# KrainskiL/CGE.jl

Measured on AMD Instinct MI355X. Metric: edge_alpha_evals_per_sec, higher is better.
Workload: dtype f64

## Files before the change

### cge.jl_amd/api.py

```python
from __future__ import annotations

import atexit
import ctypes as C
import os
import sys
import weakref

import numpy as np

from .args import _SplitRule

_HERE = os.path.dirname(os.path.abspath(__file__))
_LIB_PATH = os.path.join(_HERE, "csrc", "build", "libcge_hip.so")
_lib = None

CGE_OK = 0
_CODES = {-1: "AssertionError", -2: "ErrorException: Trying to split homogenous cluster",
          -3: "ErrorException: Unexpected empty cluster generated", -4: "HIP error / no GPU",
          -5: "collective hook failed", -6: "out of memory", -7: "bad argument"}


class CGEError(RuntimeError):
    def __init__(self, code, msg=""):
        super().__init__(f"{_CODES.get(code, 'error')} (code {code}){': ' + msg if msg else ''}")
# ... 991 lines not shown
    def set_collectives(self, fn, rank, world):
        cb = ALLREDUCE_FN(fn)
        coll = Collectives(cb, None, rank, world)
        self._keep = [cb, coll]
        self._check(self.L.cge_set_collectives(self.h, C.byref(coll)))

    def set_collectives_ext(self, allgather=None, reduce_scatter=None):
        ag = GATHER_FN(allgather) if allgather else GATHER_FN()
        rs = GATHER_FN(reduce_scatter) if reduce_scatter else GATHER_FN()
        ext = CollectivesExt(ag, rs)
        self._keep = list(getattr(self, "_keep", [])) + [ag, rs, ext]
        self._check(self.L.cge_set_collectives_ext(self.h, C.byref(ext)))

    def clear_collectives(self):
        self._check(self.L.cge_comm_finalize(self.h))
        self._check(self.L.cge_set_collectives(self.h, None))
        self._keep = []

    def init_rccl(self, unique_id: bytes, rank: int, world: int):
        assert len(unique_id) == 128
        buf = C.create_string_buffer(bytes(unique_id), 128)
        self._check(self.L.cge_comm_init_rccl(self.h, buf, C.c_int(rank), C.c_int(world)))

    def finalize_rccl(self):
        self._check(self.L.cge_comm_finalize(self.h))

    def rccl_selftest(self, arr, op=0):
        a = np.ascontiguousarray(arr).copy()
        assert a.dtype.itemsize == 8
        self._check(self.L.cge_rccl_selftest(self.h, _p(a), C.c_int64(a.size), C.c_int(op)))
        return a

    def louvain(self):
        out = np.zeros(self.n, dtype=np.int64)
        nc, q, rounds = C.c_int64(), C.c_double(), C.c_int64()
        self._check(self.L.cge_louvain(self.h, _p(out), C.byref(nc), C.byref(q), C.byref(rounds)))
        return out, nc.value, q.value, rounds.value

    def louvain_levels(self, max_levels=0):
        count, cap = C.c_int64(), (int(max_levels) if 0 < int(max_levels) < 8 else 8)
        while True:
            comm = np.zeros((cap, self.n), dtype=np.int64)
            nc, q, rounds = np.zeros(cap, dtype=np.int64), np.zeros(cap), np.zeros(cap, dtype=np.int64)
            rc = self.L.cge_louvain_levels(self.h, C.c_int64(int(max_levels)), C.c_int64(cap), _p(comm), C.byref(count), _p(nc),
                                           _p(q), _p(rounds))
            if rc == -7 and count.value > cap:
                cap = count.value
                continue
            self._check(rc)
            break
        return [(comm[l], int(nc[l]), float(q[l]), int(rounds[l])) for l in range(count.value)]

    _TEST_OPTIONS = ("louvain_wave_len", "fit_persistent_test_delay", "fit_persistent_test_timeout", "test_bvec_plain", "test_rss2_one_kernel",
                     "exact_resident_limit")

    def set_option(self, key, value):
        if key in self._TEST_OPTIONS:
            self._check(self.L.cge_set_test_option(self.h, key.encode(), C.c_int64(int(value))))
            return
        self._check(self.L.cge_set_option(self.h, key.encode(), C.c_int64(int(value))))

    def get_stat(self, key):
        v = C.c_int64()
        self._check(self.L.cge_get_stat(self.h, key.encode(), C.byref(v)))
        return v.value

    def last_diameter(self):
        import struct

        hi = struct.unpack("d", struct.pack("q", self.get_stat("diameter_bits")))[0]
        return hi, {1: "brute", 2: "pruned"}.get(self.get_stat("diameter_path"), "none"), \
            self.get_stat("diameter_candidate_pairs"), self.get_stat("diameter_candidate_tiles")

    def profile_enable(self, on=True):
        self._check(self.L.cge_profile_enable(self.h, C.c_int(int(on))))

    def profile_select(self, names=()):
        self._check(self.L.cge_profile_select(self.h, ",".join(names).encode()))

    def profile_reset(self):
        self._check(self.L.cge_profile_reset(self.h))

    def profile(self):
        buf = C.create_string_buffer(4096)
        self._check(self.L.cge_profile_names(self.h, buf, C.c_int64(4096)))
        res = {}
        for name in filter(None, buf.value.decode().split(",")):
            n, ms = C.c_int64(), C.c_double()
            self._check(self.L.cge_profile_get(self.h, name.encode(), C.byref(n), C.byref(ms)))
            res[name] = {"launches": n.value, "total_ms": ms.value}
        return res

    def phase_ms(self):
        res = {}
        buf = C.create_string_buffer(4096)
        self._check(self.L.cge_phase_names(self.h, buf, C.c_int64(4096)))
        for ph in filter(None, buf.value.decode().split(",")):
            ms = C.c_double()
            self._check(self.L.cge_phase_ms(self.h, ph.encode(), C.byref(ms)))
            res[ph] = ms.value
        return res


_default_ctx = None


def default_context():
# ... 96 lines not shown
```

### cge.jl_amd/csrc/capi.cpp

```cpp
#include "common.hpp"
#include "../../include/cge_hip_testing.h"

void flush_timers(cge_ctx *c) {
    for (auto &kv : c->timers) {
        for (auto &pr : kv.second.pending) {
            float ms = 0.f;
            (void)hipEventSynchronize(pr.second);
            if (hipEventElapsedTime(&ms, pr.first, pr.second) == hipSuccess) kv.second.total_ms += ms;
            c->event_pool.push_back(pr.first);
            c->event_pool.push_back(pr.second);
        }
        kv.second.pending.clear();
    }
}
template <class Map>
static int key_names(const Map &m, char *buf, int64_t buf_len) {
    std::string s;
    for (auto &kv : m) s += (s.empty() ? "" : ",") + kv.first;
    snprintf(buf, (size_t)buf_len, "%s", s.c_str());
    return CGE_OK;
}

extern "C" {

// ... 230 lines not shown
int cge_louvain(cge_ctx *c, int64_t *comm_out, int64_t *n_comm, double *modularity, int64_t *rounds) {
    if (!c || !comm_out) return CGE_E_ARG;
    CGE_TRY_ON_DEVICE(c)
    if (!c->src.p || c->m <= 0 || c->n <= 0) CGE_THROW(CGE_E_ARG, "louvain: no resident graph (cge_set_graph)");
    if (c->edges_sharded) CGE_THROW(CGE_E_ARG, "louvain: the resident edge list is sharded over the ranks (option shard_ingest)");
    k_louvain_level1(c, comm_out, n_comm, modularity, rounds);
    CGE_CATCH(c)
}
int cge_louvain_levels(cge_ctx *c, int64_t max_levels, int64_t levels_cap, int64_t *comm_out, int64_t *n_levels, int64_t *n_comm,
                       double *modularity, int64_t *rounds) {
    if (!c || !n_levels || levels_cap < 0) return CGE_E_ARG;
    if (levels_cap > 0 && (!comm_out || !n_comm || !modularity || !rounds)) return CGE_E_ARG;
    CGE_TRY_ON_DEVICE(c)
    if (!c->src.p || c->m <= 0 || c->n <= 0) CGE_THROW(CGE_E_ARG, "louvain: no resident graph (cge_set_graph)");
    if (c->edges_sharded) CGE_THROW(CGE_E_ARG, "louvain: the resident edge list is sharded over the ranks (option shard_ingest)");
    *n_levels = k_louvain_levels(c, max_levels, levels_cap, comm_out, n_comm, modularity, rounds);
    if (levels_cap > 0 && *n_levels > levels_cap)
        CGE_THROW(CGE_E_ARG, "louvain: the hierarchy has %lld levels, the caller's arrays hold %lld", (long long)*n_levels,
                  (long long)levels_cap);
    CGE_CATCH(c)
}

int cge_set_option(cge_ctx *c, const char *key, int64_t value) {
    if (!c || !key) return CGE_E_ARG;
    const auto is = [&](const char *k) { return !strcmp(key, k); };
    const auto ranged = [&](auto &field, int64_t lo, int64_t hi) {
        if (value < lo || value > hi) return (int)CGE_E_ARG;
        field = (std::remove_reference_t<decltype(field)>)value;
        return (int)CGE_OK;
    };
    const auto flag = [&](auto &field) { field = value != 0; return (int)CGE_OK; };
    if (is("diameter")) return ranged(c->opt_diameter, 0, 2);
    if (is("diameter_f32")) return ranged(c->opt_diameter_f32, 0, 2);
    if (is("fit_persistent")) return ranged(c->opt_fit_persistent, 0, 2);
    if (is("pow_exp2")) return flag(c->opt_pow_exp2);
    if (is("shard_runsplit")) return ranged(c->opt_shard_forced, 0, 2);
    if (is("shard_samples")) return ranged(c->opt_shard_samples, 0, 2);
    if (is("exact_relabel")) return flag(c->opt_exact_relabel);
    if (is("bvec_blocks")) return flag(c->opt_bvec_blocks);
    if (is("wedges_reduce_scatter")) return flag(c->opt_wedges_rs);
    if (is("fit_fused")) return flag(c->opt_fit_fused);
    if (is("shard_ingest")) return flag(c->opt_shard_ingest);
    if (is("shard_rows")) return flag(c->opt_shard_rows);
    if (is("landmark_edges")) return flag(c->opt_landmark_edges);
    if (is("exact_packed")) return ranged(c->opt_exact_packed, 0, 1);
    if (is("fit_max_iterations")) return ranged(c->opt_fit_max_iters, 1, INT64_MAX);
    return CGE_E_ARG;
}
int cge_set_test_option(void *ctx, const char *key, int64_t value) {
    cge_ctx *c = (cge_ctx *)ctx;
    if (!c || !key) return CGE_E_ARG;
    if (!strcmp(key, "test_bvec_plain")) { c->opt_test_bvec_plain = value != 0; return CGE_OK; }
    if (!strcmp(key, "test_rss2_one_kernel")) { c->opt_test_rss2_one_kernel = value != 0; return CGE_OK; }
    if (!strcmp(key, "fit_persistent_test_delay") && value >= 0 && value <= 100000) { c->opt_fit_test_delay = (int)value; return CGE_OK; }
    if (!strcmp(key, "fit_persistent_test_timeout")) { c->opt_fit_test_timeout = value != 0; return CGE_OK; }
    if (!strcmp(key, "louvain_wave_len") && value >= -2 && value <= INT32_MAX) { c->opt_test_louvain_wave_len = value; return CGE_OK; }
    if (!strcmp(key, "exact_resident_limit") && value >= 0) { c->opt_test_resident_limit = (double)value; return CGE_OK; }
    return CGE_E_ARG;
}
int cge_get_stat(cge_ctx *c, const char *key, int64_t *value) {
    if (!c || !key || !value) return CGE_E_ARG;
    if (!strcmp(key, "landmarks")) *value = c->lm_ready ? c->N : 0;
    else if (!strcmp(key, "diameter_path")) *value = c->stat_diameter_path;
    else if (!strcmp(key, "diameter_candidate_pairs")) *value = c->stat_cand_pairs;
    else if (!strcmp(key, "diameter_candidate_tiles")) *value = c->stat_cand_tiles;
    else if (!strcmp(key, "diameter_refs")) *value = c->stat_nref;
    else if (!strcmp(key, "diameter_bound_pass")) *value = c->stat_bound_pass;
    else if (!strcmp(key, "diameter_arg_i")) *value = c->stat_hi_i + 1;
    else if (!strcmp(key, "diameter_arg_j")) *value = c->stat_hi_j + 1;
    else if (!strcmp(key, "fit_persistent_alphas")) *value = c->stat_fit_persistent;
    else if (!strcmp(key, "fit_iterations")) *value = c->stat_fit_iters;
    else if (!strcmp(key, "exact_packed")) *value = c->stat_exact_packed;
    else if (!strcmp(key, "exact_matrix_bytes")) *value = c->stat_exact_matrix_bytes;
    else if (!strcmp(key, "fit_fused_alphas")) *value = c->stat_fit_fused;
    else if (!strcmp(key, "fit_persistent_fallbacks")) *value = c->stat_fit_fallbacks;
    else if (!strcmp(key, "fit_batched_launches")) *value = c->stat_fit_batched_launches;
    else if (!strcmp(key, "fit_batched_alphas")) *value = c->stat_fit_batched_alphas;
    else if (!strcmp(key, "landmark_batches")) *value = c->stat_lm_batches;
    else if (!strcmp(key, "landmark_batch_rows")) *value = c->stat_lm_rows;
    else if (!strcmp(key, "landmark_splits")) *value = c->stat_lm_splits;
    else if (!strcmp(key, "cut_tie_tasks")) {
        int v = 0;
        if (c->cut_ties.p && (hipStreamSynchronize(c->stream) != hipSuccess ||
                              hipMemcpy(&v, c->cut_ties.p, sizeof(int), hipMemcpyDeviceToHost) != hipSuccess))
            return CGE_E_HIP;
        *value = v;
    }
    else if (!strcmp(key, "edge_layout_build_us")) *value = c->stat_layout_build_us;
    else if (!strcmp(key, "edge_chunks")) *value = c->be_nchunks;
    else if (!strcmp(key, "edges_resident")) *value = c->m;
    else if (!strcmp(key, "edges_total")) *value = c->m_total;
    else if (!strcmp(key, "embedding_words_resident")) *value = (i64)c->Xr.n;
    else if (!strcmp(key, "rows_resident")) *value = c->Xr.p ? lm_rows(c) : 0;
    else if (!strcmp(key, "rows_total")) *value = c->n;
    else if (!strcmp(key, "collective_calls")) *value = c->stat_coll_calls;
    else if (!strcmp(key, "collective_bytes")) *value = c->stat_coll_bytes;
    else if (!strcmp(key, "diameter_bits")) memcpy(value, &c->stat_last_hi, sizeof(double));
    else return CGE_E_ARG;
    return CGE_OK;
}

int cge_profile_enable(cge_ctx *c, int on) {
    if (!c) return CGE_E_ARG;
    c->profiling = on != 0;
    return CGE_OK;
}
// ... 254 lines not shown
```

### cge.jl_amd/csrc/common.hpp

```cpp
#pragma once
#include <hip/hip_runtime.h>

#include <algorithm>
#include <atomic>
#include <chrono>
#include <condition_variable>
#include <functional>
#include <mutex>
#include <thread>
#include <cstdint>
#include <cstdio>
#include <cstdlib>
#include <cstring>
#include <map>
#include <memory>
#include <string>
#include <vector>

#include "../../include/cge_hip.h"

typedef int64_t i64;
typedef int32_t i32;

struct MaxRec {
// ... 298 lines not shown
    DevBuf<double> lemb;
    DevBuf<double> lweight, dii;
    DevBuf<i32> lcomm;
    DevBuf<double> wedges;
    DevBuf<double> vectC;
    i64 n_ledges = 0;
    bool wedges_ready = false;

    DevBuf<double> s_emb, s_dist, s_vw, s_vectC, s_degin, s_degout;
    DevBuf<i32> s_comm;
    DevBuf<double> auc_part, js_part;
    DevBuf<unsigned> js_counter;
    unsigned js_launches = 0;
    DevBuf<double> sw_D, sw_GD, sw_T1, sw_T2, sw_S1, sw_S2, sw_rowbins, sw_vectB, sw_scal, sw_lohi, sw_fitstate, sw_mm;
    DevBuf<int> sw_flags;
    DevBuf<unsigned long long> sw_fring;
    DevBuf<double> sw_PK;
    int opt_exact_packed = 0;
    double opt_test_resident_limit = 0;
    i64 stat_exact_packed = 0;
    i64 stat_exact_matrix_bytes = 0;
    bool sweep_used_fp_P = false;
    DevBuf<double> fp_T, fp_Tsave, fp_P, fp_fpart, fp_Td, fp_flow;
    DevBuf<double> ls_eigscr;
    bool bvec_contig = false;
    bool bvec_blocks = false;
    int opt_bvec_blocks = 0;
    DevBuf<i32> sw_bt_fc, sw_bt_ns, sw_bt_base;
    i64 flow_armed_words = 0;
    DevBuf<double> sw_bt_part;
    DevBuf<i32> sw_bt_desc;
    DevBuf<double> sw_fused_pw;
    DevBuf<char> sw_fused_epi;
    int opt_fit_fused = 1;
    i64 stat_fit_fused = 0;
    DevBuf<double> batch_scal, batch_vectB, batch_jspart, batch_flow;
    PinBuf<double> batch_pin;
    i64 stat_fit_batched_launches = 0, stat_fit_batched_alphas = 0;
    DevBuf<i32> sw_rl_order, sw_rl_comm;
    DevBuf<double> sw_rl_emb, sw_rl_vec, sw_rl_T;
    DevBuf<int> fp_flags;
    PinBuf<double> pin_scal;
    hipEvent_t sweep_ev[2] = {nullptr, nullptr};
    int opt_pow_exp2 = 1;
    i64 pow_logs_N = 0;
    bool pow_logs_upper = false;
    i64 pow_logs_blocked_N = 0;
    DevBuf<double> sw_Lh;
    DevBuf<float> sw_Ll;
    bool opt_exact_relabel = true;
    int opt_shard_samples = 1;
    int opt_shard_forced = 1;
    int opt_test_rss2_one_kernel = 0;
    i64 opt_test_louvain_wave_len = -2;
    int opt_test_bvec_plain = 0;
    int opt_fit_persistent = 0;
    i64 opt_fit_max_iters = 2000000;
    int opt_fit_test_timeout = 0;
    int opt_fit_test_delay = 0;
    i64 stat_lm_batches = 0, stat_lm_rows = 0, stat_lm_splits = 0;
    DevBuf<int> cut_ties;
    i64 stat_fit_persistent = 0;
    i64 stat_fit_iters = 0;
    bool fit_persistent_broken = false;
    i64 stat_fit_fallbacks = 0;
    int fit_fallback_streak = 0;
    i64 fit_skip_sweeps = 0;
    DevBuf<i32> sw_cm_off, sw_cm_mem, sw_cm_pos;
    DevBuf<double> sw_zeros, sw_zsum;
    DevBuf<MaxRec> mp_recs;
    DevBuf<i64> mp_count;
    DevBuf<int2> nt_pairs, nt_tiles;
    DevBuf<i32> nt_idx;
    DevBuf<double> nt_out, nt_rows;
    DevBuf<double> mp_rd2, mp_refmu;
    DevBuf<double> mp_commax;
    DevBuf<int2> mp_plist;
    DevBuf<i32> mp_lref, mp_refoff, mp_refmem;
    DevBuf<double> gmean;
    bool emb_nonfinite = false;
    DevBuf<double> Xs, rns, Ms, mnorm, Pm;
    DevBuf<double> pc_groups;
    DevBuf<float> Xs32, Ms32;
    DevBuf<unsigned short> Xb16, Mb16;
    DevBuf<int> dm_flag;
    DevBuf<double> xe, xe_rns, dm_seed;
    DevBuf<i32> xe_pos, xe_glob, xe_sub, dm_soffE;
    int opt_diameter_f32 = 2;
    DevBuf<i32> pos2node, sub_land, dm_soff, dm_memoff, dm_mem;
    DevBuf<BoundRec> bound_list;
    DevBuf<int2> tile_list;
    std::vector<i32> h_mem_off, h_mem;
    DevBuf<uint64_t> uniq_hash;
    DevBuf<unsigned long long> uniq_table;
    int opt_diameter = 0;
    i64 stat_cand_pairs = 0, stat_cand_tiles = 0;
    int stat_diameter_path = 0;
    double stat_last_hi = 0.0;
    i64 stat_hi_i = -1, stat_hi_j = -1;
    int stat_bound_pass = 0;
    i64 stat_nref = 0;
    DevBuf<i32> ls_rows, ls_row_task, ls_ct, ls_cb, ls_ce, ls_co, ls_tco;
    DevBuf<double> ls_part, ls_mean, ls_sw, ls_cov, ls_vec, ls_z, ls_sums;
    DevBuf<unsigned char> ls_side, ls_state;
    DevBuf<double> ls_params;
    PinBuf<double> pin_sums, pin_params;
// ... 557 lines not shown
```

### cge.jl_amd/csrc/kernels_lm.hip

```cpp
#include "common.hpp"
#include <type_traits>
#include "mfma_tile.hpp"

#define WAVE 64

template <int CTRL>
__device__ __forceinline__ double dpp_move(double v) {
    const long long b = __double_as_longlong(v);
    const int lo = __builtin_amdgcn_update_dpp(0, (int)(unsigned)b, CTRL, 0xf, 0xf, false);
    const int hi = __builtin_amdgcn_update_dpp(0, (int)(unsigned)(b >> 32), CTRL, 0xf, 0xf, false);
    return __longlong_as_double(((long long)hi << 32) | (unsigned)lo);
}
__device__ __forceinline__ double lane_value(double v, int lane) {
    const long long b = __double_as_longlong(v);
    const int lo = __builtin_amdgcn_readlane((int)(unsigned)b, lane);
    const int hi = __builtin_amdgcn_readlane((int)(unsigned)(b >> 32), lane);
    return __longlong_as_double(((long long)hi << 32) | (unsigned)lo);
}
__device__ __forceinline__ double wave_allsum(double v) {
    v += dpp_move<0xB1>(v);
    v += dpp_move<0x4E>(v);
    v += dpp_move<0x141>(v);
    v += dpp_move<0x140>(v);
    return ((lane_value(v, 0) + lane_value(v, 16)) + lane_value(v, 32)) + lane_value(v, 48);
// ... 1764 lines not shown
    asm volatile("v_fmac_f64_dpp %0, %1, -%2 row_newbcast:%3 row_mask:0xf bank_mask:0xf" : "+v"(acc) : "v"(bc), "v"(a), "n"(N));
}
template <int NG>
__device__ __forceinline__ void dpp_fence(double (&v)[NG]) {
    if constexpr (NG == 1) asm volatile("s_nop 1" : "+v"(v[0]));
    else asm volatile("s_nop 1" : "+v"(v[0]), "+v"(v[NG - 1]));
}
template <int JJ, int NR, int NC, int R0 = 0>
struct EigCols {
    static constexpr int NG = (NC + 15) / 16;
    static __device__ __forceinline__ void matvec(double (&s)[NR], const double (&a)[NR][NC], const double (&uc)[NG]) {
#pragma unroll
        for (int r = R0; r < NR; r++) fmac_bcast<JJ % 16>(s[r], uc[JJ / 16], a[r][JJ]);
        EigCols<JJ + 1, NR, NC, R0>::matvec(s, a, uc);
    }
    static __device__ __forceinline__ void rank2(double (&a)[NR][NC], const double (&uc)[NG], const double (&wc)[NG],
                                                 const double (&u)[NR], const double (&w)[NR]) {
#pragma unroll
        for (int r = R0; r < NR; r++) {
            fnmac_bcast<JJ % 16>(a[r][JJ], uc[JJ / 16], w[r]);
            fnmac_bcast<JJ % 16>(a[r][JJ], wc[JJ / 16], u[r]);
        }
        EigCols<JJ + 1, NR, NC, R0>::rank2(a, uc, wc, u, w);
    }
};
template <int NR, int NC, int R0>
struct EigCols<NC, NR, NC, R0> {
    static constexpr int NG = (NC + 15) / 16;
    static __device__ __forceinline__ void matvec(double (&)[NR], const double (&)[NR][NC], const double (&)[NG]) {}
    static __device__ __forceinline__ void rank2(double (&)[NR][NC], const double (&)[NG], const double (&)[NG], const double (&)[NR],
                                                 const double (&)[NR]) {}
};
template <int NR, int NC>
__device__ __forceinline__ void eig_pick_column(const double (&a)[NR][NC], int jj, double (&v)[NR]) {
#define EP_CASE(J)                                                                                                          \
    case J:                                                                                                                 \
        if constexpr (J < NC) {                                                                                             \
            _Pragma("unroll") for (int r = 0; r < NR; r++) v[r] = a[r][J];                                                  \
        }                                                                                                                   \
        break;
#pragma unroll
    for (int r = 0; r < NR; r++) v[r] = 0.0;
    switch (jj) {
        EP_CASE(0) EP_CASE(1) EP_CASE(2) EP_CASE(3) EP_CASE(4) EP_CASE(5) EP_CASE(6) EP_CASE(7)
        EP_CASE(8) EP_CASE(9) EP_CASE(10) EP_CASE(11) EP_CASE(12) EP_CASE(13) EP_CASE(14) EP_CASE(15)
        EP_CASE(16) EP_CASE(17) EP_CASE(18) EP_CASE(19) EP_CASE(20) EP_CASE(21) EP_CASE(22) EP_CASE(23)
        EP_CASE(24) EP_CASE(25) EP_CASE(26) EP_CASE(27) EP_CASE(28) EP_CASE(29) EP_CASE(30) EP_CASE(31)
    default: break;
    }
#undef EP_CASE
}
template <int NR, int NC, bool DPPF>
__global__ __launch_bounds__(256, 2) void group_eig_kernel(const double *__restrict__ cov, int d,
                                                           double *__restrict__ vec, int diag_stage) {
    constexpr int DP = 64 * NR;
    __shared__ __attribute__((aligned(16))) double X[DP], U[DP], W[DP], Pp[4][DP], V[DP];
    __shared__ __attribute__((aligned(16))) double diag[DP], off[DP], beta[DP], V0[DP], tri[4 * DP], red[32];
    const int tid = threadIdx.x, lane = tid & 63, wv = __builtin_amdgcn_readfirstlane(tid >> 6);
    const double *src = cov + (size_t)blockIdx.x * d * d;
    double *out = vec + (size_t)blockIdx.x * d;
    if (d == 1) {
        if (tid == 0) out[0] = 1.0;
        return;
    }
    double a[NR][NC];
#pragma unroll
    for (int r = 0; r < NR; r++) {
        const int row = lane + 64 * r;
#pragma unroll
        for (int jj = 0; jj < NC; jj++) {
            const int col = NC * wv + jj;
            a[r][jj] = (row < d && col < d) ? src[(size_t)col * d + row] : 0.0;
        }
    }
    auto extract = [&](int kn, auto) {
        if (wv == kn / NC) {
            double v[NR];
            eig_pick_column<NR, NC>(a, kn % NC, v);
#pragma unroll
            for (int r = 0; r < NR; r++) X[lane + 64 * r] = v[r];
        }
    };
    using RBlk0 = std::integral_constant<int, 0>;
    using RBlkL = std::integral_constant<int, NR - 1>;
    if (tid < DP) { beta[tid] = 0.0; off[tid] = 0.0; V0[tid] = 0.0; X[tid] = 0.0; }
    __syncthreads();
    extract(0, RBlk0{});
#ifdef CGE_EIG_CLOCK
    unsigned long long ck_acc[8] = {0, 0, 0, 0, 0, 0, 0, 0}, ck_t = __builtin_amdgcn_s_memtime();
#define CK(j) { const unsigned long long ck_n = __builtin_amdgcn_s_memtime(); ck_acc[j] += ck_n - ck_t; ck_t = ck_n; }
#else
#define CK(j)
#endif
    auto hh_step = [&](const int k, auto r0c) {
        constexpr int R0 = decltype(r0c)::value;
        asm volatile("s_waitcnt lgkmcnt(0)" ::: "memory");
        __syncthreads();
        CK(0)
        const int o = k + 1;
        double x[NR], u[NR];
        double part = 0.0;
#pragma unroll
        for (int r = 0; r < NR; r++) {
            const int row = lane + 64 * r;
            x[r] = (row > k) ? X[row] : 0.0;
            part += (row > o) ? x[r] * x[r] : 0.0;
        }
        constexpr int NG = (NC + 15) / 16;
        double uc[NG], wc[NG];
        if (DPPF) {
#pragma unroll
            for (int g = 0; g < NG; g++) {
                const int col = NC * wv + 16 * g + (lane & 15);
                uc[g] = (col > k && col < DP) ? X[col < DP ? col : 0] : 0.0;
            }
        }
        const double alpha = X[o];
        if (tid == 0) diag[k] = X[k];
        const double sigma = wave_allsum(part);
        CK(1)
        const bool refl = sigma != 0.0;
        double mu, v0r, bpr;
        if (diag_stage == 13) { mu = alpha + sigma; v0r = alpha - mu; bpr = sigma * 0.5; }
        else if (diag_stage == 11) {
            mu = sqrt(alpha * alpha + sigma);
            v0r = (alpha <= 0.0) ? alpha - mu : -sigma * fast_rcp(alpha + mu);
            bpr = 2.0 * fast_rcp(sigma + v0r * v0r);
        } else {
            mu = sqrt(alpha * alpha + sigma);
            v0r = (alpha <= 0.0) ? alpha - mu : -sigma / (alpha + mu);
            bpr = 2.0 / (sigma + v0r * v0r);
        }
        const double v0 = refl ? v0r : 0.0;
        const double bp = refl ? bpr : 0.0;
        CK(2)
        if (tid == 0) { beta[k] = bp; off[k] = refl ? mu : alpha; V0[k] = v0; }
#pragma unroll
        for (int r = 0; r < NR; r++) {
            const int row = lane + 64 * r;
            u[r] = (row == o) ? v0 : x[r];
            if (!DPPF) U[row] = u[r];
        }
        if (DPPF) {
#pragma unroll
            for (int g = 0; g < NG; g++)
                if (NC * wv + 16 * g + (lane & 15) == o) uc[g] = v0;
            dpp_fence(uc);
        }
        __builtin_amdgcn_wave_barrier();
        const bool live = NC * wv + NC > o && diag_stage != 10;
        {
            double s[NR];
#pragma unroll
            for (int r = 0; r < NR; r++) s[r] = 0.0;
            if (DPPF) {
                if (live) EigCols<0, NR, NC, R0>::matvec(s, a, uc);
            } else if (live) {
#pragma unroll
                for (int jj = 0; jj < NC; jj++) {
                    if (jj % 8 == 0) asm volatile("" ::: "memory");
                    const double uj = U[NC * wv + jj];
#pragma unroll
                    for (int r = R0; r < NR; r++) s[r] = fma(a[r][jj], uj, s[r]);
                }
            }
#pragma unroll
            for (int r = 0; r < NR; r++) Pp[wv][lane + 64 * r] = s[r];
        }
        CK(3)
        __syncthreads();
        CK(4)
        double w[NR];
        part = 0.0;
#pragma unroll
        for (int r = 0; r < NR; r++) {
            const int row = lane + 64 * r;
            w[r] = bp * (((Pp[0][row] + Pp[1][row]) + Pp[2][row]) + Pp[3][row]);
            part += w[r] * u[r];
        }
        const double K = 0.5 * bp * wave_allsum(part);
#pragma unroll
        for (int r = 0; r < NR; r++) {
            const int row = lane + 64 * r;
            w[r] = (row >= o) ? w[r] - K * u[r] : 0.0;
            W[row] = w[r];
        }
        __builtin_amdgcn_wave_barrier();
        CK(5)
        if (DPPF) {
            if (diag_stage != 10) {
#pragma unroll
                for (int g = 0; g < NG; g++) {
                    const int col = NC * wv + 16 * g + (lane & 15);
                    wc[g] = W[col < DP ? col : 0];
                }
                dpp_fence(wc);
                EigCols<0, NR, NC, R0>::rank2(a, uc, wc, u, w);
            }
        } else if (diag_stage != 10) {
#pragma unroll
            for (int jj = 0; jj < NC; jj++) {
                if (jj % 8 == 0) asm volatile("" ::: "memory");
                const double uj = U[NC * wv + jj], wj = W[NC * wv + jj];
#pragma unroll
                for (int r = R0; r < NR; r++) a[r][jj] = fma(-u[r], wj, fma(-w[r], uj, a[r][jj]));
            }
        }
        CK(6)
        extract(k + 1, r0c);
        CK(7)
    };
    {
        int k = 0;
        if constexpr (NR > 1) {
            for (; k + 2 < d && k + 1 < 64; k++) hh_step(k, RBlk0{});
            for (; k + 2 < d; k++) hh_step(k, RBlkL{});
        } else {
            for (; k + 2 < d; k++) hh_step(k, RBlk0{});
        }
    }
#ifdef CGE_EIG_CLOCK
    if (blockIdx.x == 0 && lane == 0 && (wv == 0 || wv == 3))
        printf("eig clock wave %d: barrier_a %llu  reads+sigma %llu  sqrt/div %llu  matvec+Pp %llu  barrier_b %llu  w %llu  rank2 %llu  extract %llu (s_memtime ticks over %d steps)\n",
               wv, ck_acc[0], ck_acc[1], ck_acc[2], ck_acc[3], ck_acc[4], ck_acc[5], ck_acc[6], ck_acc[7], d - 2);
#endif
#undef CK
    __syncthreads();
    if (tid == 0) { diag[d - 2] = X[d - 2]; off[d - 2] = X[d - 1]; }
    __syncthreads();
    if (NR > 1 && d - 1 >= 64) extract(d - 1, RBlkL{});
    else extract(d - 1, RBlk0{});
    __syncthreads();
    if (tid == 0) diag[d - 1] = X[d - 1];
    __syncthreads();
    if (diag_stage == 1) { if (tid < d) out[tid] = diag[tid]; return; }
    double glo = 1e300, ghi = -1e300, gn = 0.0;
    if (tid < d) {
        const double rad = (tid > 0 ? fabs(off[tid - 1]) : 0.0) + (tid + 1 < d ? fabs(off[tid]) : 0.0);
        glo = diag[tid] - rad;
        ghi = diag[tid] + rad;
        gn = fabs(diag[tid]) + rad;
        tri[tid] = tid > 0 ? off[tid - 1] * off[tid - 1] : 0.0;
    }
    for (int o2 = 32; o2 > 0; o2 >>= 1) {
        glo = fmin(glo, __shfl_xor(glo, o2));
        ghi = fmax(ghi, __shfl_xor(ghi, o2));
        gn = fmax(gn, __shfl_xor(gn, o2));
    }
    double *gs = red + 8;
    if (lane == 0) { gs[wv * 3] = glo; gs[wv * 3 + 1] = ghi; gs[wv * 3 + 2] = gn; }
// ... 518 lines not shown
            if (bk == 0.0) continue;
            const double sc = bk * block_sum_512(vk * yt, red);
            yt -= sc * vk;
        }
        panel_sync();
        if (tid < d) v[tid] = yt;
        panel_sync();
    }
    double part = 0.0, best = -1.0;
    int bi = 0;
    for (int i = tid; i < d; i += EWP_T) {
        const double t = v[i];
        part += t * t;
        if (fabs(t) > best) { best = fabs(t); bi = i; }
    }
    double nrm = sqrt(block_sum_512(part, red));
    const bool degenerate = !(nrm > 0.0) || !(nrm < 1e300);
    for (int o2 = 32; o2 > 0; o2 >>= 1) {
        const double ob = __shfl_xor(best, o2);
        const int oi = __shfl_xor(bi, o2);
        if (ob > best || (ob == best && oi < bi)) { best = ob; bi = oi; }
    }
    panel_sync();
    if (lane == 0) { misc[2 * wv] = best; misc[2 * wv + 1] = (double)bi; }
    panel_sync();
    best = misc[0];
    bi = (int)misc[1];
    for (int w2 = 1; w2 < 8; w2++) {
        const double ob = misc[2 * w2];
        const int oi = (int)misc[2 * w2 + 1];
        if (ob > best || (ob == best && oi < bi)) { best = ob; bi = oi; }
    }
    if (degenerate) {
        for (int i = tid; i < d; i += EWP_T) out[i] = (i == 0) ? 1.0 : 0.0;
        return;
    }
    const double sg = ((v[bi] < 0.0) ? -1.0 : 1.0) / nrm;
    for (int i = tid; i < d; i += EWP_T) out[i] = v[i] * sg;
}
bool k_group_eig(cge_ctx *c, const double *cov, i64 n_tasks, i64 d, double *vec) {
    if (d > 512) return false;
    if (d > 128) {
        ScopedKernelTimer t(c, "group_eig");
        const size_t plds = (size_t)(2 * EWP_NB * d + d + 8 + 8 * 2 * EWP_NB + 2 * EWP_NB + 32) * sizeof(double);
        cge_allow_lds((const void *)group_eig_panel_kernel, 160 * 1024);
        c->ls_eigscr.ensure((size_t)n_tasks * EWP_SCR);
        hipLaunchKernelGGL(group_eig_panel_kernel, dim3((unsigned)n_tasks), dim3(EWP_T), plds, c->stream,
                           const_cast<double *>(cov), (int)d, vec, c->ls_eigscr.p);
        return true;
    }
    ScopedKernelTimer t(c, "group_eig");
    static const int diag_stage = getenv("CGE_EIG_DIAG") ? atoi(getenv("CGE_EIG_DIAG")) : 0;
    const dim3 grid((unsigned)n_tasks), block(256);
    if (d <= 32) hipLaunchKernelGGL((group_eig_kernel<1, 8, true>), grid, block, 0, c->stream, cov, (int)d, vec, diag_stage);
    else if (d <= 64) hipLaunchKernelGGL((group_eig_kernel<1, 16, true>), grid, block, 0, c->stream, cov, (int)d, vec, diag_stage);
    else hipLaunchKernelGGL((group_eig_kernel<2, 32, true>), grid, block, 0, c->stream, cov, (int)d, vec, diag_stage);
    return true;
}

__global__ __launch_bounds__(256) void group_project_kernel(const double *__restrict__ Xr, const double *__restrict__ vw,
                                                            const i32 *__restrict__ rows, const i32 *__restrict__ row_task,
                                                            i64 n_rows, i64 d, const double *__restrict__ mean,
                                                            const double *__restrict__ vec, double *__restrict__ z) {
    constexpr int PR = 16;
    const i64 j0 = (((i64)blockIdx.x * blockDim.x + threadIdx.x) / WAVE) * PR;
    const int lane = threadIdx.x & 63;
    if (j0 >= n_rows) return;
    if (d <= 128) {
        const i64 jl = (j0 + (lane & 15) < n_rows) ? j0 + (lane & 15) : n_rows - 1;
        const i32 vrow = rows[jl], trow = row_task[jl];
        const double sqv = sqrt(vw[vrow]);
        const bool hb = lane + 64 < d, ha = lane < d;
        double xa[PR], xb[PR];
#pragma unroll
        for (int u = 0; u < PR; u++) {
            const i64 v = __builtin_amdgcn_readlane(vrow, u);
            const double *x = Xr + v * d;
            xa[u] = ha ? x[lane] : 0.0;
            xb[u] = hb ? x[lane + 64] : 0.0;
        }
        int cur = __builtin_amdgcn_readlane(trow, 0);
        double ma, mb, ea, eb;
        {
            const double *mu = mean + (i64)cur * d, *ev = vec + (i64)cur * d;
            ma = ha ? mu[lane] : 0.0; ea = ha ? ev[lane] : 0.0;
            mb = hb ? mu[lane + 64] : 0.0; eb = hb ? ev[lane + 64] : 0.0;
        }
        double zs = 0.0;
#pragma unroll
        for (int u = 0; u < PR; u++) {
            const int t = __builtin_amdgcn_readlane(trow, u);
            if (t != cur) {
                cur = t;
                const double *mu = mean + (i64)cur * d, *ev = vec + (i64)cur * d;
                ma = ha ? mu[lane] : 0.0; ea = ha ? ev[lane] : 0.0;
                mb = hb ? mu[lane + 64] : 0.0; eb = hb ? ev[lane + 64] : 0.0;
            }
            const double sq = lane_value(sqv, u);
            double s = 0.0;
            if (ha) s = fma((xa[u] - ma) * sq, ea, s);
            if (hb) s = fma((xb[u] - mb) * sq, eb, s);
            s = wave_tree_sum_lane0(s);
            const double s0 = lane_value(s, 0);
            if (lane == u) zs = s0;
        }
        if (lane < PR && j0 + lane < n_rows) z[j0 + lane] = zs;
        return;
    }
    if (d <= 512) {
// ... 467 lines not shown
```

Baseline: 11.84 billion.

## Reassign eigensolver wave roles by SIMD placement and overlap reflector math with matvec

```diff
diff --git a/cge.jl_amd/api.py b/cge.jl_amd/api.py
--- a/cge.jl_amd/api.py
+++ b/cge.jl_amd/api.py
@@ -1067,7 +1067,7 @@
         return [(comm[l], int(nc[l]), float(q[l]), int(rounds[l])) for l in range(count.value)]
 
     _TEST_OPTIONS = ("louvain_wave_len", "fit_persistent_test_delay", "fit_persistent_test_timeout", "test_bvec_plain", "test_rss2_one_kernel",
-                     "exact_resident_limit")
+                     "exact_resident_limit", "test_eig_roles")
 
     def set_option(self, key, value):
         if key in self._TEST_OPTIONS:
diff --git a/cge.jl_amd/csrc/capi.cpp b/cge.jl_amd/csrc/capi.cpp
--- a/cge.jl_amd/csrc/capi.cpp
+++ b/cge.jl_amd/csrc/capi.cpp
@@ -306,6 +306,7 @@
     if (!c || !key) return CGE_E_ARG;
     if (!strcmp(key, "test_bvec_plain")) { c->opt_test_bvec_plain = value != 0; return CGE_OK; }
     if (!strcmp(key, "test_rss2_one_kernel")) { c->opt_test_rss2_one_kernel = value != 0; return CGE_OK; }
+    if (!strcmp(key, "test_eig_roles") && value >= 0 && value <= 3) { c->opt_test_eig_roles = (int)value; return CGE_OK; }
     if (!strcmp(key, "fit_persistent_test_delay") && value >= 0 && value <= 100000) { c->opt_fit_test_delay = (int)value; return CGE_OK; }
     if (!strcmp(key, "fit_persistent_test_timeout")) { c->opt_fit_test_timeout = value != 0; return CGE_OK; }
     if (!strcmp(key, "louvain_wave_len") && value >= -2 && value <= INT32_MAX) { c->opt_test_louvain_wave_len = value; return CGE_OK; }
diff --git a/cge.jl_amd/csrc/common.hpp b/cge.jl_amd/csrc/common.hpp
--- a/cge.jl_amd/csrc/common.hpp
+++ b/cge.jl_amd/csrc/common.hpp
@@ -374,6 +374,7 @@
     int opt_shard_samples = 1;
     int opt_shard_forced = 1;
     int opt_test_rss2_one_kernel = 0;
+    int opt_test_eig_roles = 0;
     i64 opt_test_louvain_wave_len = -2;
     int opt_test_bvec_plain = 0;
     int opt_fit_persistent = 0;
diff --git a/cge.jl_amd/csrc/kernels_lm.hip b/cge.jl_amd/csrc/kernels_lm.hip
--- a/cge.jl_amd/csrc/kernels_lm.hip
+++ b/cge.jl_amd/csrc/kernels_lm.hip
@@ -1840,17 +1840,33 @@
 }
 template <int NR, int NC, bool DPPF>
 __global__ __launch_bounds__(256, 2) void group_eig_kernel(const double *__restrict__ cov, int d,
-                                                           double *__restrict__ vec, int diag_stage) {
+                                                           double *__restrict__ vec, int diag_stage, int roles) {
     constexpr int DP = 64 * NR;
     __shared__ __attribute__((aligned(16))) double X[DP], U[DP], W[DP], Pp[4][DP], V[DP];
     __shared__ __attribute__((aligned(16))) double diag[DP], off[DP], beta[DP], V0[DP], tri[4 * DP], red[32];
-    const int tid = threadIdx.x, lane = tid & 63, wv = __builtin_amdgcn_readfirstlane(tid >> 6);
+    __shared__ int place[4];
+    const int lane = threadIdx.x & 63, pw = __builtin_amdgcn_readfirstlane(threadIdx.x >> 6);
     const double *src = cov + (size_t)blockIdx.x * d * d;
     double *out = vec + (size_t)blockIdx.x * d;
     if (d == 1) {
-        if (tid == 0) out[0] = 1.0;
+        if (threadIdx.x == 0) out[0] = 1.0;
         return;
     }
+    if (lane == 0) place[pw] = (int)__builtin_amdgcn_s_getreg(4 | (31 << 11)) & 0x3f;
+    if (threadIdx.x < DP) { beta[threadIdx.x] = 0.0; off[threadIdx.x] = 0.0; V0[threadIdx.x] = 0.0; X[threadIdx.x] = 0.0; }
+    __syncthreads();
+    int role = roles == 2 ? 3 - pw : roles == 3 ? (pw + 1) & 3 : pw;
+    if (roles == 0) {
+        const int p0 = place[0], p1 = place[1], p2 = place[2], p3 = place[3];
+        const int simds = (1 << (p0 >> 4)) | (1 << (p1 >> 4)) | (1 << (p2 >> 4)) | (1 << (p3 >> 4));
+        if (simds == 15) {
+            const int on0 = (p0 >> 4) == 0 ? p0 : (p1 >> 4) == 0 ? p1 : (p2 >> 4) == 0 ? p2 : p3;
+            const int mine = place[pw] >> 4;
+            role = (on0 & 1) ? 3 - mine : mine;
+        }
+    }
+    const int wv = __builtin_amdgcn_readfirstlane(role), tid = 64 * wv + lane;
+    __builtin_amdgcn_s_setprio(2);
     double a[NR][NC];
 #pragma unroll
     for (int r = 0; r < NR; r++) {
@@ -1871,8 +1887,6 @@
     };
     using RBlk0 = std::integral_constant<int, 0>;
     using RBlkL = std::integral_constant<int, NR - 1>;
-    if (tid < DP) { beta[tid] = 0.0; off[tid] = 0.0; V0[tid] = 0.0; X[tid] = 0.0; }
-    __syncthreads();
     extract(0, RBlk0{});
 #ifdef CGE_EIG_CLOCK
     unsigned long long ck_acc[8] = {0, 0, 0, 0, 0, 0, 0, 0}, ck_t = __builtin_amdgcn_s_memtime();
@@ -1908,42 +1922,39 @@
         const double sigma = wave_allsum(part);
         CK(1)
         const bool refl = sigma != 0.0;
-        double mu, v0r, bpr;
-        if (diag_stage == 13) { mu = alpha + sigma; v0r = alpha - mu; bpr = sigma * 0.5; }
-        else if (diag_stage == 11) {
-            mu = sqrt(alpha * alpha + sigma);
-            v0r = (alpha <= 0.0) ? alpha - mu : -sigma * fast_rcp(alpha + mu);
-            bpr = 2.0 * fast_rcp(sigma + v0r * v0r);
+        const bool live = NC * wv + NC > o && diag_stage != 10;
+        const bool owner = DPPF && o / NC == wv;
+        double s[NR];
+#pragma unroll
+        for (int r = 0; r < NR; r++) s[r] = 0.0;
+        if (DPPF && live && !owner) {
+            dpp_fence(uc);
+            EigCols<0, NR, NC, R0>::matvec(s, a, uc);
+        }
+        double mu = 0.0, v0r = 0.0;
+        if (owner || wv == 0 || !DPPF) {
+            if (diag_stage == 13) { mu = alpha + sigma; v0r = alpha - mu; }
+            else {
+                mu = sqrt(alpha * alpha + sigma);
+                if (diag_stage == 11) v0r = (alpha <= 0.0) ? alpha - mu : -sigma * fast_rcp(alpha + mu);
+                else v0r = (alpha <= 0.0) ? alpha - mu : -sigma / (alpha + mu);
+            }
+        }
+        CK(2)
+        if (DPPF) {
+            if (live && owner) {
+                const double v0o = refl ? v0r : 0.0;
+#pragma unroll
+                for (int g = 0; g < NG; g++)
+                    if (NC * wv + 16 * g + (lane & 15) == o) uc[g] = v0o;
+                dpp_fence(uc);
+                EigCols<0, NR, NC, R0>::matvec(s, a, uc);
+            }
         } else {
-            mu = sqrt(alpha * alpha + sigma);
-            v0r = (alpha <= 0.0) ? alpha - mu : -sigma / (alpha + mu);
-            bpr = 2.0 / (sigma + v0r * v0r);
-        }
-        const double v0 = refl ? v0r : 0.0;
-        const double bp = refl ? bpr : 0.0;
-        CK(2)
-        if (tid == 0) { beta[k] = bp; off[k] = refl ? mu : alpha; V0[k] = v0; }
-#pragma unroll
-        for (int r = 0; r < NR; r++) {
-            const int row = lane + 64 * r;
-            u[r] = (row == o) ? v0 : x[r];
-            if (!DPPF) U[row] = u[r];
-        }
-        if (DPPF) {
-#pragma unroll
-            for (int g = 0; g < NG; g++)
-                if (NC * wv + 16 * g + (lane & 15) == o) uc[g] = v0;
-            dpp_fence(uc);
-        }
-        __builtin_amdgcn_wave_barrier();
-        const bool live = NC * wv + NC > o && diag_stage != 10;
-        {
-            double s[NR];
-#pragma unroll
-            for (int r = 0; r < NR; r++) s[r] = 0.0;
-            if (DPPF) {
-                if (live) EigCols<0, NR, NC, R0>::matvec(s, a, uc);
-            } else if (live) {
+#pragma unroll
+            for (int r = 0; r < NR; r++) U[lane + 64 * r] = (lane + 64 * r == o) ? (refl ? v0r : 0.0) : x[r];
+            __builtin_amdgcn_wave_barrier();
+            if (live) {
 #pragma unroll
                 for (int jj = 0; jj < NC; jj++) {
                     if (jj % 8 == 0) asm volatile("" ::: "memory");
@@ -1952,12 +1963,22 @@
                     for (int r = R0; r < NR; r++) s[r] = fma(a[r][jj], uj, s[r]);
                 }
             }
-#pragma unroll
-            for (int r = 0; r < NR; r++) Pp[wv][lane + 64 * r] = s[r];
+        }
+#pragma unroll
+        for (int r = 0; r < NR; r++) Pp[wv][lane + 64 * r] = s[r];
+        if (wv == 0) {
+            double bpr;
+            if (diag_stage == 13) bpr = sigma * 0.5;
+            else if (diag_stage == 11) bpr = 2.0 * fast_rcp(sigma + v0r * v0r);
+            else bpr = 2.0 / (sigma + v0r * v0r);
+            if (tid == 0) { beta[k] = refl ? bpr : 0.0; off[k] = refl ? mu : alpha; V0[k] = refl ? v0r : 0.0; }
         }
         CK(3)
         __syncthreads();
         CK(4)
+        const double bp = beta[k], v0 = V0[k];
+#pragma unroll
+        for (int r = 0; r < NR; r++) u[r] = (lane + 64 * r == o) ? v0 : x[r];
         double w[NR];
         part = 0.0;
 #pragma unroll
@@ -1976,14 +1997,16 @@
         __builtin_amdgcn_wave_barrier();
         CK(5)
         if (DPPF) {
-            if (diag_stage != 10) {
+            if (live) {
 #pragma unroll
                 for (int g = 0; g < NG; g++) {
                     const int col = NC * wv + 16 * g + (lane & 15);
                     wc[g] = W[col < DP ? col : 0];
                 }
                 dpp_fence(wc);
+                __builtin_amdgcn_s_setprio(0);
                 EigCols<0, NR, NC, R0>::rank2(a, uc, wc, u, w);
+                __builtin_amdgcn_s_setprio(2);
             }
         } else if (diag_stage != 10) {
 #pragma unroll
@@ -2608,9 +2631,10 @@
     ScopedKernelTimer t(c, "group_eig");
     static const int diag_stage = getenv("CGE_EIG_DIAG") ? atoi(getenv("CGE_EIG_DIAG")) : 0;
     const dim3 grid((unsigned)n_tasks), block(256);
-    if (d <= 32) hipLaunchKernelGGL((group_eig_kernel<1, 8, true>), grid, block, 0, c->stream, cov, (int)d, vec, diag_stage);
-    else if (d <= 64) hipLaunchKernelGGL((group_eig_kernel<1, 16, true>), grid, block, 0, c->stream, cov, (int)d, vec, diag_stage);
-    else hipLaunchKernelGGL((group_eig_kernel<2, 32, true>), grid, block, 0, c->stream, cov, (int)d, vec, diag_stage);
+    const int roles = c->opt_test_eig_roles;
+    if (d <= 32) hipLaunchKernelGGL((group_eig_kernel<1, 8, true>), grid, block, 0, c->stream, cov, (int)d, vec, diag_stage, roles);
+    else if (d <= 64) hipLaunchKernelGGL((group_eig_kernel<1, 16, true>), grid, block, 0, c->stream, cov, (int)d, vec, diag_stage, roles);
+    else hipLaunchKernelGGL((group_eig_kernel<2, 32, true>), grid, block, 0, c->stream, cov, (int)d, vec, diag_stage, roles);
     return true;
 }
 
diff --git a/profiles/eig_place_probe.hip b/profiles/eig_place_probe.hip
--- /dev/null
+++ b/profiles/eig_place_probe.hip
@@ -0,0 +1,109 @@
+#include <hip/hip_runtime.h>
+#include <algorithm>
+#include <cstdio>
+#include <map>
+#include <set>
+#include <vector>
+#define CHECK(x) do { hipError_t e_ = (x); if (e_ != hipSuccess) { printf("HIP error %s at line %d\n", hipGetErrorString(e_), __LINE__); return 1; } } while (0)
+struct Rec { unsigned hw, xcc; unsigned long long t0, t1; };
+constexpr int NWG = 512;
+constexpr int GETREG_HW_ID = 4 | (0 << 6) | (31 << 11);
+constexpr int GETREG_XCC_ID = 20 | (0 << 6) | (31 << 11);
+__global__ __launch_bounds__(256, 2) void place_kernel(Rec *__restrict__ out, int naps) {
+    __shared__ double lds[1996];
+    const int tid = threadIdx.x, lane = tid & 63, wave = tid >> 6;
+    const unsigned long long t0 = __builtin_amdgcn_s_memtime();
+    const unsigned hw = __builtin_amdgcn_s_getreg(GETREG_HW_ID), xcc = __builtin_amdgcn_s_getreg(GETREG_XCC_ID);
+    asm volatile("v_mov_b32 v223, 0" ::: "v223");
+    for (int i = tid; i < 1996; i += 256) lds[i] = (double)i;
+    __syncthreads();
+    for (int i = 0; i < naps; i++) __builtin_amdgcn_s_sleep(127);
+    __syncthreads();
+    const unsigned long long t1 = __builtin_amdgcn_s_memtime();
+    if (lane == 0) {
+        Rec r = {hw, xcc, t0, t1};
+        if (lds[wave] < 0.0) r.hw = 0;
+        out[blockIdx.x * 4 + wave] = r;
+    }
+}
+int main() {
+    Rec *d;
+    std::vector<Rec> h(NWG * 4);
+    CHECK(hipMalloc(&d, h.size() * sizeof(Rec)));
+    for (int rep = 0; rep < 2; rep++) {
+        CHECK(hipMemset(d, 0, h.size() * sizeof(Rec)));
+        hipLaunchKernelGGL(place_kernel, dim3(NWG), dim3(256), 0, 0, d, 30);
+        CHECK(hipGetLastError());
+        CHECK(hipDeviceSynchronize());
+    }
+    CHECK(hipMemcpy(h.data(), d, h.size() * sizeof(Rec), hipMemcpyDeviceToHost));
+    unsigned all_or = 0, all_and = ~0u;
+    std::set<unsigned> waveid, simd, cu, sh, se, xcc;
+    for (const Rec &r : h) {
+        all_or |= r.hw; all_and &= r.hw;
+        waveid.insert(r.hw & 15); simd.insert((r.hw >> 4) & 3); cu.insert((r.hw >> 8) & 15); sh.insert((r.hw >> 12) & 1);
+        se.insert((r.hw >> 13) & 7); xcc.insert(r.xcc & 15);
+    }
+    printf("HW_ID bits that vary over %d waves: 0x%08x (or 0x%08x, and 0x%08x)\n", NWG * 4, all_or & ~all_and, all_or, all_and);
+    auto show = [](const char *n, const std::set<unsigned> &s) { printf("  %s:", n); for (unsigned v : s) printf(" %u", v); printf("\n"); };
+    show("WAVE_ID [3:0]", waveid); show("SIMD_ID [5:4]", simd); show("CU_ID [11:8]", cu); show("SH_ID [12]", sh);
+    show("SE_ID [15:13]", se); show("XCC_ID (reg 20) [3:0]", xcc);
+    printf("first 8 workgroups, waves 0..3 as simd.slot (cu key = xcc/se/sh/cu):\n");
+    auto cukey = [&](const Rec &r) { return ((r.xcc & 15) << 16) | (r.hw & 0xff00); };
+    for (int g = 0; g < 8; g++) {
+        printf("  wg %3d key %05x:", g, cukey(h[g * 4]));
+        for (int w = 0; w < 4; w++) printf(" %u.%u", (h[g * 4 + w].hw >> 4) & 3, h[g * 4 + w].hw & 15);
+        printf("\n");
+    }
+    int distinct = 0, same_cu = 0, same_slot = 0, same_parity = 0;
+    std::map<std::vector<unsigned>, int> orders;
+    for (int g = 0; g < NWG; g++) {
+        std::set<unsigned> s;
+        std::vector<unsigned> ord;
+        bool cu_ok = true, slot_ok = true, par_ok = true;
+        for (int w = 0; w < 4; w++) {
+            const Rec &r = h[g * 4 + w];
+            s.insert((r.hw >> 4) & 3); ord.push_back((r.hw >> 4) & 3);
+            cu_ok &= cukey(r) == cukey(h[g * 4]);
+            slot_ok &= (r.hw & 15) == (h[g * 4].hw & 15);
+            par_ok &= (r.hw & 1) == (h[g * 4].hw & 1);
+        }
+        distinct += s.size() == 4; same_cu += cu_ok; same_slot += slot_ok; same_parity += par_ok;
+        orders[ord]++;
+    }
+    printf("workgroups of %d: four different SIMDs %d, all waves on one CU %d, one slot number in all four waves %d, one slot parity %d\n",
+           NWG, distinct, same_cu, same_slot, same_parity);
+    printf("SIMD of waves 0,1,2,3 -> workgroups:\n");
+    for (auto &kv : orders) printf("  %u %u %u %u : %d\n", kv.first[0], kv.first[1], kv.first[2], kv.first[3], kv.second);
+    std::map<unsigned, std::vector<int>> by_cu;
+    for (int g = 0; g < NWG; g++) by_cu[cukey(h[g * 4])].push_back(g);
+    printf("CUs that ran workgroups: %zu\n", by_cu.size());
+    int pairs = 0, w3_same = 0, w0_same = 0, w03_cross = 0, slot_par_diff = 0, printed = 0;
+    std::map<std::pair<unsigned, unsigned>, int> slots;
+    for (auto &kv : by_cu)
+        for (size_t i = 0; i < kv.second.size(); i++)
+            for (size_t j = i + 1; j < kv.second.size(); j++) {
+                const int a = kv.second[i], b = kv.second[j];
+                const unsigned long long lo = std::max(h[a * 4].t0, h[b * 4].t0), hi = std::min(h[a * 4].t1, h[b * 4].t1);
+                if (hi <= lo || 2 * (hi - lo) < h[a * 4].t1 - h[a * 4].t0) continue;
+                pairs++;
+                auto sd = [&](int g, int w) { return (h[g * 4 + w].hw >> 4) & 3; };
+                w3_same += sd(a, 3) == sd(b, 3); w0_same += sd(a, 0) == sd(b, 0);
+                w03_cross += sd(a, 0) == sd(b, 3) || sd(a, 3) == sd(b, 0);
+                slot_par_diff += ((h[a * 4].hw ^ h[b * 4].hw) & 1) != 0;
+                slots[{std::min(h[a * 4].hw & 15, h[b * 4].hw & 15), std::max(h[a * 4].hw & 15, h[b * 4].hw & 15)}]++;
+                if (printed++ < 12) {
+                    printf("  cu %05x: wg %3d", kv.first, a);
+                    for (int w = 0; w < 4; w++) printf(" %u.%u", sd(a, w), h[a * 4 + w].hw & 15);
+                    printf("  | wg %3d", b);
+                    for (int w = 0; w < 4; w++) printf(" %u.%u", sd(b, w), h[b * 4 + w].hw & 15);
+                    printf("\n");
+                }
+            }
+    printf("co-resident pairs %d: waves 3 on one SIMD %d, waves 0 on one SIMD %d, a wave 0 with the other's wave 3 %d, slot parity differs %d\n",
+           pairs, w3_same, w0_same, w03_cross, slot_par_diff);
+    printf("slot numbers (wave 0's) of the two workgroups of a pair -> pairs:\n");
+    for (auto &kv : slots) printf("  %u %u : %d\n", kv.first.first, kv.first.second, kv.second);
+    CHECK(hipFree(d));
+    return 0;
+}
diff --git a/profiles/eig_stage_split.py b/profiles/eig_stage_split.py
--- /dev/null
+++ b/profiles/eig_stage_split.py
@@ -0,0 +1,31 @@
+import os
+import sys
+
+import numpy as np
+
+sys.path.insert(0, os.path.dirname(os.path.dirname(os.path.abspath(__file__))))
+from cge.jl_amd import api
+
+api._LIB_PATH = os.path.join(os.path.dirname(api._LIB_PATH), sys.argv[1])
+d, Ts, REPS = int(sys.argv[2]), [int(t) for t in sys.argv[3:]], 5
+ctx = api.Context()
+roles = os.environ.get("CGE_EIG_SPLIT_ROLES")
+if roles is not None:
+    ctx.set_option("test_eig_roles", int(roles))
+ctx.profile_enable(True)
+for T in Ts:
+    rng = np.random.default_rng(0)
+    A = np.empty((T, d, d))
+    for t in range(T):
+        Y = rng.normal(size=(2 * d, d)) * rng.uniform(0.5, 2.0, size=d)
+        A[t] = Y.T @ Y
+    ctx.group_eig(A)
+    ms = []
+    for _ in range(REPS):
+        ctx.profile_reset()
+        for _ in range(10):
+            ctx.group_eig(A)
+        pr = ctx.profile()["group_eig"]
+        ms.append(pr["total_ms"] / pr["launches"])
+    print(f"{sys.argv[1]} roles={roles} CGE_EIG_DIAG={os.environ.get('CGE_EIG_DIAG', '0')} T={T} d={d}: ms per launch "
+          + " ".join(f"{m:.4f}" for m in ms) + f"  min {min(ms):.4f} max {max(ms):.4f}", flush=True)
```

New measurement: 12.10 billion, median of 6. 1.02x the previous value.
